# daviddmc/NeSVoR

Measured on AMD Instinct MI355X. Metric: INR train iters/sec (2^20 samples, L=16 hash, 64-wide MLP), higher is better.
Workload: dtype f32 (MLP products evaluated on 2-way fp16 splits of the power-of-two-scaled fp32 operands, fp32 accumulation: error against fp64 at or below the fp32 MFMA chain's; the all-fp32-MFMA rate of the same run is in strict_fp32_mfma)

## Files before the change

include/nesvor_hip.h:

```cpp
#ifndef NESVOR_HIP_H
#define NESVOR_HIP_H

#include <stdint.h>

#ifdef __cplusplus
extern "C" {
#endif

#define NESVOR_MAX_LEVELS 32
#define NESVOR_MAX_MLP_LAYERS 4

int nesvor_hip_abi_version(void);

int nesvor_axisangle2mat_forward(const float* ax, float* mat, int n, void* stream);
int nesvor_axisangle2mat_backward(const float* grad_mat, const float* ax, float* grad_ax, int n, void* stream);
int nesvor_mat2axisangle_forward(const float* mat, float* ax, int n, void* stream);
int nesvor_mat2axisangle_backward(const float* mat, const float* grad_ax, float* grad_mat, int n, void* stream);
int nesvor_axisangle2mat_forward_f64(const double* ax, double* mat, int n, void* stream);
int nesvor_axisangle2mat_backward_f64(const double* grad_mat, const double* ax, double* grad_ax, int n, void* stream);
int nesvor_mat2axisangle_forward_f64(const double* mat, double* ax, int n, void* stream);
int nesvor_mat2axisangle_backward_f64(const double* mat, const double* grad_ax, double* grad_mat, int n, void* stream);

int nesvor_trans_loss(const float* ax, const float* ax_init, float* loss_per_slice, float* grad_ax, int n, void* stream);

// ... 36 lines not shown
                                         const double* psf, const double* grad_slices, const uint8_t* slices_mask,
                                         double* grad_vol, double* grad_transforms, int D, int H, int W, int d_p, int h_p,
                                         int w_p, int n, int h, int w, double res_slice, void* stream);
int nesvor_slice_acq_adjoint_backward_interp_f64(const double* transforms, double* grad_vol, const double* vol_weight,
                                                 const uint8_t* vol_mask, const double* psf, const double* slices,
                                                 const uint8_t* slices_mask, const double* vol, double* grad_slices,
                                                 double* grad_transforms, int D, int H, int W, int d_p, int h_p, int w_p,
                                                 int n, int h, int w, double res_slice, int equalize, void* stream);
int nesvor_slice_acq_forward_f64(const double* transforms, const double* vol, const uint8_t* vol_mask,
                                 const uint8_t* slices_mask, const double* psf, double* slices, double* slices_weight,
                                 int D, int H, int W, int d_p, int h_p, int w_p, int n, int h, int w,
                                 double res_slice, int interp_psf, void* stream);
int nesvor_slice_acq_adjoint_forward_f64(const double* transforms, const double* psf, const double* slices,
                                         const uint8_t* slices_mask, const uint8_t* vol_mask, double* vol, double* vol_weight,
                                         double* scratch, int D, int H, int W, int d_p, int h_p, int w_p, int n, int h, int w,
                                         double res_slice, int equalize, void* stream);
int nesvor_slice_acq_backward_f64(const double* transforms, const double* vol, const uint8_t* vol_mask, const double* psf,
                                  const double* grad_slices, const uint8_t* slices_mask, double* grad_vol,
                                  double* grad_transforms, double* scratch, int D, int H, int W, int d_p, int h_p, int w_p,
                                  int n, int h, int w, double res_slice, void* stream);
int nesvor_slice_acq_adjoint_backward_f64(const double* transforms, double* grad_vol, const double* vol_weight,
                                          const uint8_t* vol_mask, const double* psf, const double* slices,
                                          const uint8_t* slices_mask, const double* vol, double* grad_slices,
                                          double* grad_transforms, int D, int H, int W, int d_p, int h_p, int w_p, int n, int h,
                                          int w, double res_slice, int equalize, void* stream);

typedef struct {
  int32_t n_levels;
  int32_t n_features;
  float scale[NESVOR_MAX_LEVELS];
  uint32_t res[NESVOR_MAX_LEVELS];
  uint32_t size[NESVOR_MAX_LEVELS];
  uint32_t offset[NESVOR_MAX_LEVELS];
  uint32_t hashed[NESVOR_MAX_LEVELS];
} nesvor_grid_t;

#define NESVOR_LAYOUT_ROW_MAJOR 0
#define NESVOR_LAYOUT_FEATURE_MAJOR 1
#define NESVOR_LAYOUT_CLUSTERED 4
#define NESVOR_LAYOUT_UNCLUSTERED 8
#define NESVOR_LAYOUT_DY_SCRATCH 16
#define NESVOR_LAYOUT_MASK 3

int nesvor_hashgrid_forward(const nesvor_grid_t* grid, const float* u, const float* table, float* pe,
                            int64_t N, int layout, void* stream);
int nesvor_hashgrid_forward_bounded(const nesvor_grid_t* grid, const float* u, const float* table, float* pe,
                                    int64_t N, int layout, float* pe_absmax, void* stream);
int64_t nesvor_hashgrid_forward_workspace_bytes(const nesvor_grid_t* grid, int64_t N, int layout);
int nesvor_hashgrid_forward_unclustered(const nesvor_grid_t* grid, const float* u, const float* table, float* pe, int64_t N,
                                        int layout, float* pe_absmax, void* workspace, int64_t workspace_bytes, void* stream);
int64_t nesvor_hashgrid_backward_workspace_bytes(const nesvor_grid_t* grid, int64_t N, const float* queue_scale);
int64_t nesvor_hashgrid_backward_workspace_bytes_ex(const nesvor_grid_t* grid, int64_t N, const float* queue_scale, int layout);
int64_t nesvor_hashgrid_backward_workspace_zero_bytes(void);
int64_t nesvor_hashgrid_backward_overflow_offset(void* workspace);
int nesvor_hashgrid_backward(const nesvor_grid_t* grid, const float* u, const float* table, const float* dpe,
                             float* grad_table, float* grad_u, int64_t N, int layout, void* workspace, int stages,
                             const float* queue_scale, void* stream);

int nesvor_hashgrid_backward_levels(const nesvor_grid_t* grid, const float* u, const float* table, const float* dpe,
                                    float* grad_table, float* grad_u, int64_t N, int layout, void* workspace, int stages,
                                    int level_begin, int level_end, const float* queue_scale, void* stream);
int nesvor_hashgrid_backward_bounded(const nesvor_grid_t* grid, const float* u, const float* table, const float* dpe,
                                     float* grad_table, float* grad_u, int64_t N, int layout, void* workspace, int stages,
                                     int level_begin, int level_end, const float* queue_scale, const float* dy_bound,
                                     void* stream);
int nesvor_hashgrid_backward_atomic(const nesvor_grid_t* grid, const float* u, const float* table, const float* dpe,
                                    float* grad_table, float* grad_u, int64_t N, int layout, void* stream);

int nesvor_psf_transform_forward(const float* mat, const int64_t* slice_idx, const float* xyz, const float* sigma,
                                 const float* noise, const float* bb, float* x, float* u, int B, int S, void* stream);
int nesvor_psf_transform_backward(const float* mat, const int64_t* slice_idx, const float* xyz, const float* sigma,
                                  const float* noise, const float* bb, const float* dx, const float* du, float* dmat,
                                  int B, int S, void* stream);
int nesvor_psf_transform_forward_rng(const float* mat, const int64_t* slice_idx, const float* xyz, const float* sigma,
                                     uint64_t seed, uint64_t offset, const float* bb, float* x, float* u, int B, int S,
                                     void* stream);
int nesvor_psf_transform_forward_rng_gather(const float* mat, const int64_t* slice_idx, const float* xyz, const float* sigma,
                                            uint64_t seed, uint64_t offset, const float* bb, float* x, float* u, int B, int S,
                                            const float* embedding, float* se, int ks, void* stream);
int nesvor_psf_transform_backward_rng(const float* mat, const int64_t* slice_idx, const float* xyz, const float* sigma,
                                      uint64_t seed, uint64_t offset, const float* bb, const float* dx, const float* du,
                                      float* dmat, int B, int S, void* stream);
int nesvor_psf_transform_backward_rng_slices(const float* mat, const int64_t* slice_idx, const float* xyz, const float* sigma,
                                             uint64_t seed, uint64_t offset, const float* bounding_box, const float* dx,
                                             const float* du, float* dpix, float* dmat_slice, int B, int S, void* stream);
int nesvor_psf_noise(uint64_t seed, uint64_t offset, float* out, int64_t n_samples, void* stream);

typedef struct {
  int32_t width;
  int32_t n_hidden;
  int32_t out_dim;
  int32_t k_a, k_b, b_row0;
  int32_t samples_per_pixel;
  int32_t dxa_group_sums;
  int32_t bf16_operands;
  int32_t compact_save;
  const float* weight[NESVOR_MAX_MLP_LAYERS];
  const float* bias[NESVOR_MAX_MLP_LAYERS];
  const float* prep;
  float* y_absmax;
  const void* weight_images;
} nesvor_mlp_t;
#define NESVOR_ABSMAX_SLOTS 16
#define NESVOR_ABSMAX_STRIDE 64
#define NESVOR_ABSMAX_FLOATS (NESVOR_ABSMAX_SLOTS * NESVOR_ABSMAX_STRIDE)
#define NESVOR_MLP_PREP_XA 0
// ... 182 lines not shown
```

nesvor_amd/_lib.py:

```python
import ctypes
import os
from ctypes import POINTER, Structure, c_double, c_float, c_int, c_int32, c_int64, c_uint32, c_uint64, c_void_p

import torch

_HERE = os.path.dirname(os.path.abspath(__file__))
LIB_PATH = os.environ.get("NESVOR_HIP_LIB") or os.path.join(_HERE, "lib", "libnesvor_hip.so")
MAX_LEVELS = 32
ABI_VERSION = 37

LAYOUT_ROW_MAJOR = 0
LAYOUT_FEATURE_MAJOR = 1
STEP_DEFER_JOIN = 8
STEP_BIAS_SUM_STOP = 16
STEP_BIAS_SUM_RESUME = 32
LAYOUT_CLUSTERED = 4
LAYOUT_UNCLUSTERED = 8
LAYOUT_DY_SCRATCH = 16


class GridT(Structure):

    _fields_ = [
        ("n_levels", c_int32),
# ... 105 lines not shown
    "nesvor_hashgrid_forward_workspace_bytes": ([POINTER(GridT), c_int64, c_int], c_int64),
    "nesvor_hashgrid_forward_unclustered": ([POINTER(GridT), _P, _P, _P, c_int64, c_int, _P, _P, c_int64, _P], c_int),
    "nesvor_hashgrid_backward_workspace_bytes": ([POINTER(GridT), c_int64, _P], c_int64),
    "nesvor_hashgrid_backward_workspace_bytes_ex": ([POINTER(GridT), c_int64, _P, c_int], c_int64),
    "nesvor_hashgrid_backward_workspace_zero_bytes": ([], c_int64),
    "nesvor_hashgrid_backward_overflow_offset": ([_P], c_int64),
    "nesvor_hashgrid_backward": ([POINTER(GridT), _P, _P, _P, _P, _P, c_int64, c_int, _P, c_int, _P, _P], c_int),
    "nesvor_hashgrid_backward_levels": ([POINTER(GridT), _P, _P, _P, _P, _P, c_int64, c_int, _P, c_int, c_int, c_int, _P, _P], c_int),
    "nesvor_hashgrid_backward_bounded": ([POINTER(GridT), _P, _P, _P, _P, _P, c_int64, c_int, _P, c_int, c_int, c_int, _P, _P, _P], c_int),
    "nesvor_hashgrid_backward_atomic": ([POINTER(GridT), _P, _P, _P, _P, _P, c_int64, c_int, _P], c_int),
    "nesvor_psf_transform_forward": ([_P] * 8 + [c_int, c_int, _P], c_int),
    "nesvor_psf_transform_backward": ([_P] * 9 + [c_int, c_int, _P], c_int),
    "nesvor_psf_transform_forward_rng_gather": ([_P] * 4 + [c_uint64, c_uint64] + [_P] * 3 + [c_int, c_int, _P, _P, c_int, _P], c_int),
    "nesvor_psf_transform_forward_rng": ([_P] * 4 + [c_uint64, c_uint64] + [_P] * 3 + [c_int, c_int, _P], c_int),
    "nesvor_psf_transform_backward_rng": ([_P] * 4 + [c_uint64, c_uint64] + [_P] * 4 + [c_int, c_int, _P], c_int),
    "nesvor_psf_transform_backward_rng_slices": ([_P] * 4 + [c_uint64, c_uint64] + [_P] * 5 + [c_int, c_int, _P], c_int),
    "nesvor_psf_noise": ([c_uint64, c_uint64, _P, c_int64, _P], c_int),
    "nesvor_mlp_compact_save_ok": ([POINTER(MlpT), c_int64], c_int),
    "nesvor_mlp_bias_free_ok": ([POINTER(MlpT), c_int64], c_int),
    "nesvor_mlp_backward_fused_ok": ([POINTER(MlpT), c_int64], c_int),
    "nesvor_mlp_prepare": ([POINTER(MlpT), _P, _P, _P, c_int64, _P, c_int, _P], c_int),
    "nesvor_mlp_prepare_weights": ([_P, _P, c_int, _P, c_int64, _P, _P], c_int),
    "nesvor_mlp_prepare_weights_images": ([_P, _P, _P, c_int, _P, c_int64, _P, _P], c_int),
    "nesvor_mlp_weight_images_bytes": ([POINTER(MlpT)], c_int64),
    "nesvor_mlp_forward": ([POINTER(MlpT), _P, _P, _P, POINTER(c_void_p), c_int64, _P], c_int),
    "nesvor_mlp_backward": (
        [POINTER(MlpT), _P, _P, _P, POINTER(c_void_p), POINTER(c_void_p), _P, _P, _P, c_int, c_int64, _P],
        c_int,
    ),
    "nesvor_mlp_backward_bounded": (
        [POINTER(MlpT), _P, _P, _P, POINTER(c_void_p), POINTER(c_void_p), _P, _P, _P, c_int, c_int64, _P, _P],
        c_int,
    ),
    "nesvor_mlp_wide_saved_floats": ([POINTER(MlpWideT), c_int64], c_int64),
    "nesvor_mlp_wide_param_count": ([POINTER(MlpWideT)], c_int),
    "nesvor_mlp_wide_forward": ([POINTER(MlpWideT), _P, _P, _P, POINTER(c_void_p), c_int64, _P], c_int),
    "nesvor_mlp_wide_backward": (
        [POINTER(MlpWideT), _P, _P, _P, POINTER(c_void_p), POINTER(c_void_p), _P, _P, _P, c_int, c_int64, _P],
        c_int,
    ),
    "nesvor_mlp_wide_backward_bounded": (
        [POINTER(MlpWideT), _P, _P, _P, POINTER(c_void_p), POINTER(c_void_p), _P, _P, _P, c_int, c_int64, _P, _P],
        c_int,
    ),
    "nesvor_imaging_loss": ([POINTER(LossT), _P], c_int),
    "nesvor_slice_grads_by_slice": ([_P] * 9 + [c_int, c_int, c_int, c_int, _P], c_int),
    "nesvor_slice_grads": ([_P] * 9 + [c_int, c_int, c_int, _P], c_int),
    "nesvor_step_prologue": ([_P] * 5 + [c_int, c_int, _P], c_int),
    "nesvor_step_prologue_pose": ([_P] * 5 + [c_int, c_int, _P, _P, _P, _P], c_int),
    "nesvor_step_epilogue": ([_P] * 6 + [c_float, _P, _P, _P, _P, c_int, c_int, c_float, c_float, _P], c_int),
    "nesvor_step_epilogue_scaled": ([_P] * 6 + [c_float, _P, _P, _P, _P, _P, c_int, c_int, c_float, c_float, _P], c_int),
    "nesvor_hashgrid_backward_adamw": ([POINTER(GridT), _P, _P, _P, _P, _P, c_int64, c_int, _P, c_int, _P, _P, _P, _P, POINTER(AdamwT), _P], c_int),
    "nesvor_hashgrid_backward_adamw_levels": ([POINTER(GridT), _P, _P, _P, _P, _P, c_int64, c_int, _P, c_int, c_int, c_int, _P, _P, _P, _P, POINTER(AdamwT), _P], c_int),
    "nesvor_hashgrid_forward_levels": ([POINTER(GridT), _P, _P, _P, c_int64, c_int, _P, c_int, c_int, _P], c_int),
    "nesvor_adamw_step": (
        [_P, _P, _P, _P, c_int64] + [c_float] * 8 + [c_int, _P],
        c_int,
    ),
    "nesvor_grad_found_inf": ([_P, c_int64, _P, _P], c_int),
    "nesvor_adamw_step_scaled": ([_P, _P, _P, _P, c_int64, c_float, c_double, c_double, c_float, c_float, c_int, c_int, _P, _P], c_int),
    "nesvor_loss_scaler_update": ([_P, _P], c_int),
    "nesvor_loss_scale_weights": ([_P, _P, c_int, _P, _P], c_int),
    "nesvor_sum_rows_multi": ([_P, _P, _P, _P, c_int, c_int, _P], c_int),
    "nesvor_sum_rows": ([_P, _P, c_int, c_int, c_int, _P], c_int),
    "nesvor_step_create": ([POINTER(StepT)], c_void_p),
    "nesvor_step_update": ([_P, POINTER(StepT)], c_int),
    "nesvor_step_destroy": ([_P], None),
    "nesvor_step_join": ([_P, _P], c_int),
    "nesvor_step_set_bias_mean_ranks": ([_P, c_int], c_int),
    "nesvor_step_set_bias_mean_event": ([_P, _P], c_int),
    "nesvor_step_timing": ([_P, c_int], c_int),
    "nesvor_step_timing_read": ([_P, _P], c_int),
    "nesvor_step_run": ([_P, _P, _P, _P, c_uint64, c_uint64, _P, c_int, c_int, POINTER(AdamwT), _P], c_int),
    "nesvor_vvr_similarity": ([_P, c_int, c_int, c_int, _P, _P, _P, _P, c_int64, c_int, _P, _P, _P], c_int),
}


def exported_symbols():
    return list(_SIGNATURES)


def load():
    global _lib
    if _lib is not None:
        return _lib
    if not os.path.exists(LIB_PATH):
        raise RuntimeError(
            f"{LIB_PATH} not found: the HIP backend has not been built. "
            "Run `python -m nesvor_amd.csrc.build` (or __graft_entry__.build()). "
            "There is no CPU fallback for the native ops."
        )
    lib = ctypes.CDLL(LIB_PATH)
    for name, (argtypes, restype) in _SIGNATURES.items():
        fn = getattr(lib, name)
        fn.argtypes = argtypes
        fn.restype = restype
    v = lib.nesvor_hip_abi_version()
    if v != ABI_VERSION:
        raise RuntimeError(f"libnesvor_hip ABI {v} != expected {ABI_VERSION}; rebuild")
    _lib = lib
    return lib


def stream_ptr(device=None):
    return c_void_p(torch.cuda.current_stream(device).cuda_stream)

# ... 60 lines not shown
```

nesvor_amd/csrc/hashgrid.hip:

```cpp
#include <hip/hip_runtime.h>
#include <mutex>
#include <type_traits>
#include <unordered_map>
#include "common.h"
#include "adam.h"
#include "../../include/nesvor_hip.h"

#ifndef NESVOR_ABLATE
#define NESVOR_ABLATE 0
#endif
#define NESVOR_ABL(bit) ((NESVOR_ABLATE & (bit)) != 0)
#ifndef NESVOR_SORT_SPAN
#define NESVOR_SORT_SPAN 256
#endif

namespace {

constexpr uint32_t kPrimeY = 2654435761u;
constexpr uint32_t kPrimeZ = 805459861u;

struct LevelParams {
  float scale;
  uint32_t res, size, offset, hashed;
};

__device__ __forceinline__ LevelParams load_level(const nesvor_grid_t& g, int level) {
  LevelParams p;
  p.scale = g.scale[level];
  p.res = g.res[level];
  p.size = g.size[level];
  p.offset = g.offset[level];
  p.hashed = g.hashed[level];
  return p;
}

__device__ __forceinline__ uint32_t corner_index(const LevelParams& p, uint32_t x, uint32_t y, uint32_t z) {
  if (p.hashed) {
    const uint32_t h = x ^ (y * kPrimeY) ^ (z * kPrimeZ);
    return ((p.size & (p.size - 1)) == 0) ? (h & (p.size - 1)) : (h % p.size);
  }
  uint32_t idx = x + __umul24(y, p.res) + __umul24(z, p.res * p.res);
  if (idx >= p.size) idx %= p.size;
  return idx;
}

__device__ __forceinline__ uint32_t scan32_u32(uint32_t v, int lane) {
#define NESVOR_SCAN_STEP_(SHR)                                                                        \
  v += (uint32_t)__builtin_amdgcn_update_dpp(0, (int)v, 0x110 | (SHR), 0xf, 0xf, true);
  NESVOR_SCAN_STEP_(1) NESVOR_SCAN_STEP_(2) NESVOR_SCAN_STEP_(4) NESVOR_SCAN_STEP_(8)
#undef NESVOR_SCAN_STEP_
  const uint32_t row0 = (uint32_t)__builtin_amdgcn_readlane((int)v, 15);
  return v + ((lane >= 16 && lane < 32) ? row0 : 0u);
}
// ... 535 lines not shown
  x = (x ^ (x << 2)) & 0x09249249u;
  return x;
}

__device__ __forceinline__ unsigned long long to_fixed(float x) {
  const float t = rintf(x * 0x1p-32f);
  const int32_t lo = __float2int_rn(fmaf(-t, 0x1p32f, x));
  return ((unsigned long long)(uint32_t)((int32_t)t + (lo >> 31)) << 32) | (unsigned long long)(uint32_t)lo;
}
#ifndef NESVOR_HG_F64FIX
#define NESVOR_HG_F64FIX 0
#endif
__device__ __forceinline__ unsigned long long to_fixed51(float x, double scale) {
  return (unsigned long long)__double_as_longlong(fma((double)x, scale, 0x1.8p52));
}
__device__ __forceinline__ float from_fixed51(unsigned long long q) {
  const uint32_t lo = (uint32_t)q;
  const int32_t hi = ((int32_t)(uint32_t)(q >> 32) << 13) >> 13;
  return fmaf((float)(hi + (int32_t)(lo >> 31)), 0x1p32f, (float)(int32_t)lo);
}
__device__ __forceinline__ float from_fixed(unsigned long long q) {
  const uint32_t lo = (uint32_t)q;
  return fmaf((float)((int32_t)(q >> 32) + (int32_t)(lo >> 31)), 0x1p32f, (float)(int32_t)lo);
}


#ifndef NESVOR_FIXED32
#define NESVOR_FIXED32 0
#endif

#ifndef NESVOR_HG_SLOTS
#define NESVOR_HG_SLOTS 1024
#endif
#ifndef NESVOR_HG_MINBLOCKS
#define NESVOR_HG_MINBLOCKS 4
#endif
#ifndef NESVOR_HG_SPATIAL
#define NESVOR_HG_SPATIAL 1
#endif
#ifndef NESVOR_HG_TIMELINE
#define NESVOR_HG_TIMELINE 0
#endif
#if NESVOR_HG_TIMELINE
constexpr int kTlWgs = 64, kTlMarks = 96;
__device__ unsigned long long g_hg_timeline[kTlWgs][kTlMarks];
#define HG_TICK(site)                                                                                              \
  do {                                                                                                             \
    if (blockIdx.x < (unsigned)kTlWgs && threadIdx.x == 0 && tl_n < kTlMarks)                                      \
      g_hg_timeline[blockIdx.x][tl_n++] = ((unsigned long long)(site) << 56) | (__builtin_amdgcn_s_memtime() & 0x00FFFFFFFFFFFFFFull); \
  } while (0)
#else
#define HG_TICK(site) do { } while (0)
#endif
template <int F, int LAYOUT, bool INPUT_GRAD, bool MERGE, bool BOUND = false>
__global__ __launch_bounds__(256, F <= 2 ? NESVOR_HG_MINBLOCKS : (F == 4 ? 3 : 2)) void hashgrid_bwd_aggregate(const nesvor_grid_t g, const BwdPlan plan,
                                                              const float* __restrict__ u,
                                                              const float* __restrict__ table,
                                                              const float* __restrict__ dpe,
                                                              float* __restrict__ grad_table,
                                                              float* __restrict__ grad_u, uint32_t* __restrict__ tails,
                                                              uint32_t* __restrict__ tails_next,
                                                              uint32_t* __restrict__ records, int64_t N,
                                                              const float* __restrict__ dy_bound,
                                                              uint8_t* __restrict__ order,
                                                              int order_mode,
                                                              const uint32_t* __restrict__ perm,
                                                              int dy_by_slot) {
  for (uint32_t t = blockIdx.x * 256u + threadIdx.x; t < (uint32_t)kSubQueues * kTailStride; t += gridDim.x * 256u) tails_next[t] = 0u;
  constexpr bool kPack = (F == 2) && (NESVOR_FIXED32 != 0);
  constexpr bool kPerLevel = kPack && (NESVOR_FIXED32 >= 2);
  constexpr int kWords = kPack ? 1 : F;
  __shared__ uint32_t bcount[kMaxChunks];
  __shared__ __attribute__((aligned(16))) uint32_t bb_raw[4 * kMaxChunks];
  uint4* const bbase4 = reinterpret_cast<uint4*>(bb_raw);
  uint2(*const bbase)[kMaxChunks] = reinterpret_cast<uint2(*)[kMaxChunks]>(bb_raw);
  __shared__ uint32_t sortbuf[256];
  constexpr int kSlots = F <= 2 ? NESVOR_HG_SLOTS : (F == 4 ? 512 : 256);
  constexpr uint32_t kEmpty = 0xFFFFFFFFu;
  constexpr uint32_t kKeyMask = (1u << 27) - 1u;
  constexpr int kMaxGroup = 8;
  __shared__ __attribute__((aligned(16))) uint32_t tkeys[kSlots];
  __shared__ __attribute__((aligned(16))) unsigned long long tvals[kSlots * kWords];
  __shared__ __attribute__((aligned(16))) float tcache[INPUT_GRAD && MERGE ? kSlots * F : 1];
  __shared__ float gmax[4];
  __shared__ uint32_t lmax_bits[NESVOR_MAX_LEVELS + 1];
  __shared__ float lscale[NESVOR_MAX_LEVELS + 1][2];
  __shared__ uint32_t merge_stat[2];
  __shared__ uint32_t slots_log2;
  __shared__ uint32_t merge_off;
  __shared__ uint32_t prev_cnt;
  __shared__ float ubox[4][6];
  __shared__ uint32_t lbox[NESVOR_MAX_LEVELS + 1][8];
  __shared__ uint32_t lwin[NESVOR_MAX_LEVELS + 1];
  __shared__ uint32_t slot_off[NESVOR_MAX_LEVELS + 1], bkt_off[NESVOR_MAX_LEVELS + 1], grp_end[NESVOR_MAX_LEVELS + 1];
  __shared__ uint32_t rnd_slots[NESVOR_MAX_LEVELS + 1], rnd_bkts[NESVOR_MAX_LEVELS + 1];
  __shared__ uint32_t lpar[NESVOR_MAX_LEVELS + 1][8];
  __shared__ int32_t box_end_s;
  const int tid = threadIdx.x, lane = tid & 63;
  const int64_t base = (int64_t)blockIdx.x * 256;
  const int E = g.n_levels * F;
#if NESVOR_HG_TIMELINE
  int tl_n = 0;
  if (blockIdx.x < (unsigned)kTlWgs && tid == 0) for (int k = 0; k < kTlMarks; ++k) g_hg_timeline[blockIdx.x][k] = 0ull;
#endif
  HG_TICK(0);
  const int level_end = plan.level_end;
  const uint32_t sub = (uint32_t)__builtin_amdgcn_s_getreg((3 << 11) | (0 << 6) | 20) & (plan.n_sub - 1u);
  if (tid < kMaxChunks) bcount[tid] = 0;
  for (int t = tid; t < kSlots; t += 256) tkeys[t] = kEmpty;
  for (int t = tid; t < kSlots * kWords; t += 256) tvals[t] = 0ull;
  if (tid < 2) merge_stat[tid] = 0;
  if (tid == 0) { merge_off = MERGE ? 0u : 1u; slots_log2 = __builtin_ctz(kSlots); prev_cnt = 0u; }
  if constexpr (kPerLevel) {
    if (tid <= NESVOR_MAX_LEVELS) lmax_bits[tid] = 0u;
  }

  uint32_t sv;
  {
    const int64_t s0_ = base + tid;
    uint32_t code = 0x00ffffffu;
    if (s0_ < N) {
      const int64_t i0 = perm != nullptr ? (int64_t)perm[s0_] : s0_;
      const LevelParams pf = load_level(g, g.n_levels - 1);
      const CellPos c = locate(pf, u[3 * i0], u[3 * i0 + 1], u[3 * i0 + 2]);
      code = spread3(c.gx) | (spread3(c.gy) << 1) | (spread3(c.gz) << 2);
    }
    sv = (code << 8) | (uint32_t)tid;
    if (order_mode == 2) sv = (uint32_t)order[base + tid];
    else
// ... 272 lines not shown
#pragma unroll
        for (int f = 0; f < F; ++f) {
          v[f] = (NESVOR_HG_F64FIX != 0 ? from_fixed51(w[f]) : from_fixed(w[f])) * finv;
          tvals[f * kSlots + slot] = 0ull;
        }
      }
    }
    return any;
  };

  float dy_a[F], dy_b[F];
  int level = plan.level_begin;
  load_dy(level, dy_a);
  if (level + 1 < level_end) load_dy(level + 1, dy_b);

  constexpr int NRB = kSlots / 256;
  if constexpr (MERGE) {
    auto fill_keys = [&](int ra, int rb, float (&feat)[NRB][F]) __attribute__((always_inline)) {
      const uint32_t total = sgpr(rnd_slots[ra]);
#pragma unroll
      for (int j = 0; j < NRB; ++j) {
        const uint32_t slot = (uint32_t)j * 256u + (uint32_t)tid;
#pragma unroll
        for (int f = 0; f < F; ++f) feat[j][f] = 0.f;
        if (slot < total) {
          int lv = ra;
          for (int l = ra + 1; l < rb; ++l) lv = slot >= slot_off[l] ? l : lv;
          const uint32_t local = slot - slot_off[lv];
          const uint32_t nx = lbox[lv][3] + 2u, nxy = nx * (lbox[lv][4] + 2u);
          const uint32_t z = (uint32_t)(((float)local + 0.5f) * (1.f / (float)nxy));
          const uint32_t r = local - __umul24(z, nxy);
          const uint32_t y = (uint32_t)(((float)r + 0.5f) * (1.f / (float)nx));
          LevelParams pl;
          pl.scale = 0.f; pl.res = lpar[lv][0]; pl.size = lpar[lv][1]; pl.offset = lpar[lv][2]; pl.hashed = lpar[lv][3];
          const uint32_t key = corner_index(pl, lbox[lv][0] + (r - __umul24(y, nx)), lbox[lv][1] + y, lbox[lv][2] + z);
          tkeys[slot] = ((uint32_t)lv << 27) | key;
          if constexpr (INPUT_GRAD) load_feat<F>(table + ((size_t)pl.offset + key) * F, feat[j]);
        }
      }
    };
    auto store_feat = [&](int ra, const float (&feat)[NRB][F]) __attribute__((always_inline)) {
      if constexpr (INPUT_GRAD) {
        const uint32_t total = sgpr(rnd_slots[ra]);
#pragma unroll
        for (int j = 0; j < NRB; ++j) {
          const uint32_t slot = (uint32_t)j * 256u + (uint32_t)tid;
          if (slot < total) {
#pragma unroll
            for (int f = 0; f < F; ++f) tcache[slot * F + f] = feat[j][f];
          }
        }
      }
    };
    auto insert_round = [&](int ra, int rb) __attribute__((always_inline)) {
#pragma unroll 1
      for (int lv = ra; lv < rb; ++lv) {
        uint32_t idx_unused[8], s0, nx, nxy;
        float val[8][F];
        bool tail;
        prepare(std::true_type{}, lv, dy_a, idx_unused, s0, nx, nxy, val, tail);
#pragma unroll
        for (int f = 0; f < F; ++f) dy_a[f] = dy_b[f];
        if (lv + 2 < level_end) load_dy(lv + 2, dy_b);
        const float fs_lv = scale_of((uint32_t)lv);
        if (!NESVOR_ABL(4) && tail) {
#pragma unroll
          for (int k = 0; k < 8; ++k) slot_add(s0 + (k & 1) + ((k >> 1) & 1) * nx + (k >> 2) * nxy, val[k], fs_lv);
        }
      }
    };

    if (level < box_end) {
      int ra = level, rb = (int)sgpr(grp_end[level]);
      {
        float feat[NRB][F];
        fill_keys(ra, rb, feat);
        store_feat(ra, feat);
      }
      if constexpr (INPUT_GRAD) __syncthreads();
      HG_TICK(4);
      insert_round(ra, rb);
      HG_TICK(5);
      uint32_t rkey[NRB], rmeta[NRB], rank[NRB], rmask = 0;
      float rval[NRB][F];
      bool have_prev = false;
      for (;;) {
        __syncthreads();
        HG_TICK(0x20 | ra);
        if (have_prev && !NESVOR_ABL(8)) {
#pragma unroll
          for (int j = 0; j < NRB; ++j) {
            if (!(rmask & (1u << j))) continue;
            const uint4 bb = bbase4[rmeta[j] & 0xFFu];
            const uint32_t pos = bb.x + rank[j];
            if (pos < bb.z) {
              uint32_t* r = records + ((size_t)bb.y + pos) * (1 + F);
              r[0] = rkey[j];
#pragma unroll
              for (int f = 0; f < F; ++f) r[1 + f] = __float_as_uint(rval[j][f]);
            } else {
              atomicAdd(&tails[kOverflowBase + (rmeta[j] >> 8)], 1u);
#pragma unroll
              for (int f = 0; f < F; ++f) atomicAdd(grad_table + ((size_t)lpar[rmeta[j] >> 8][2] + rkey[j]) * F + f, rval[j][f]);
            }
          }
        }
        const int na = rb, nb_ = na < box_end ? (int)sgpr(grp_end[na]) : na;
        const bool next_box = na < box_end;
        const uint32_t n_slots = sgpr(rnd_slots[ra]);
        uint32_t lk[NRB];
#pragma unroll
        for (int j = 0; j < NRB; ++j) lk[j] = tkeys[j * 256 + tid];
        float nfeat[NRB][F];
        if (next_box) {
          fill_keys(na, nb_, nfeat);
        } else {
#pragma unroll
          for (int j = 0; j < NRB; ++j) tkeys[j * 256 + tid] = kEmpty;
        }
        rmask = 0;
        uint32_t n_last = 0;
// ... 738 lines not shown
    for (int idx = tid; idx < kGatherPts * E; idx += 256) {
      const int q = idx / E, e = idx - q * E;
      if (i0 + q < N) rows[(size_t)rank[q] * E + e] = tile[q * (E + 1) + e];
    }
  }
}
__global__ __launch_bounds__(256) void scatter_pe_rows_kernel(const float* __restrict__ rows, SortBufs s, float* __restrict__ pe, int64_t N, int E) {
  extern __shared__ float tile[];
  __shared__ uint32_t rank[kGatherPts];
  const int tid = threadIdx.x;
  const int64_t i0 = (int64_t)blockIdx.x * kGatherPts;
  const bool ok = i0 + tid < N;
  if (ok) {
    const unsigned long long w = s.where[i0 + tid];
    rank[tid] = s.first[(uint32_t)(w >> 32)] + (uint32_t)w;
  }
  __syncthreads();
  if ((E & 3) == 0) {
    const int E4 = E >> 2;
    for (int idx = tid; idx < kGatherPts * E4; idx += 256) {
      const int q = idx / E4, e = (idx - q * E4) * 4;
      if (i0 + q < N) {
        const float4 v = *reinterpret_cast<const float4*>(rows + (size_t)rank[q] * E + e);
        float* t = tile + q * (E + 1) + e;
        t[0] = v.x; t[1] = v.y; t[2] = v.z; t[3] = v.w;
      }
    }
  } else {
    for (int idx = tid; idx < kGatherPts * E; idx += 256) {
      const int q = idx / E, e = idx - q * E;
      if (i0 + q < N) tile[q * (E + 1) + e] = rows[(size_t)rank[q] * E + e];
    }
  }
  __syncthreads();
  if (ok) {
    for (int e = 0; e < E; ++e) pe[(size_t)e * N + i0 + tid] = tile[tid * (E + 1) + e];
  }
}
inline int sort_points(const float* u, int64_t N, uint32_t* base, hipStream_t st) {
  const SortPlan p = sort_plan(N);
  const SortBufs s = sort_bufs(base, N, p);
  hipError_t e = hipMemsetAsync(s.count, 0, sizeof(uint32_t) * (p.n_cells + 1), st);
  if (e != hipSuccess) return (int)e;
  hipLaunchKernelGGL(sort_place_kernel, dim3((unsigned)((N + 255) / 256)), dim3(256), 0, st, u, N, p, s);
  static std::once_flag raised;
  constexpr size_t kScanLds = sizeof(uint32_t) * (32768 + 32768 / 32);
  std::call_once(raised, []() { (void)hipFuncSetAttribute(reinterpret_cast<const void*>(sort_scan_kernel), hipFuncAttributeMaxDynamicSharedMemorySize, (int)kScanLds); });
  hipLaunchKernelGGL(sort_scan_kernel, dim3(1), dim3(1024), kScanLds, st, p, s);
  const uint64_t n_threads = (uint64_t)p.n_cells * p.cap + (uint64_t)((N + 255) / 256) * 256;
  hipLaunchKernelGGL(sort_compact_kernel, dim3((unsigned)((n_threads + 255) / 256)), dim3(256), 0, st, p, s);
  return (int)hipGetLastError();
}

template <int F, int LAYOUT>
int launch_bwd_owner(const nesvor_grid_t* g, const float* u, const float* table, const float* dpe, float* gt,
                     float* gu, int64_t N, void* workspace, int stages, int level_begin, int level_end, const float* queue_scale,
                     const float* dy_bound, const OwnerAdam* adam, hipStream_t st, int hints = 0) {
  const bool unclustered = (hints & NESVOR_LAYOUT_UNCLUSTERED) != 0;
  if constexpr (LAYOUT == NESVOR_LAYOUT_FEATURE_MAJOR) {
    if (unclustered && (hints & NESVOR_LAYOUT_DY_SCRATCH) && (stages & 1))
      return launch_bwd_owner<F, NESVOR_LAYOUT_ROW_MAJOR>(g, u, table, dpe, gt, gu, N, workspace, stages, level_begin, level_end, queue_scale,
                                                          dy_bound, adam, st, hints | 0x10000);
  }
  BwdPlan plan;
  uint64_t n_rec;
  if (!make_plan(g, N, &plan, &n_rec, queue_scale)) return (int)hipErrorInvalidValue;
  plan.level_begin = level_begin; plan.level_end = level_end;
  plan.accumulate_u = (stages & 8) ? 1 : 0;
  const int par = tails_parity(workspace, (stages & 1) && !(stages & 4));
  uint32_t* tails = reinterpret_cast<uint32_t*>(reinterpret_cast<char*>(workspace) + (par ? kTailBytes : 0));
  uint32_t* tails_next = reinterpret_cast<uint32_t*>(reinterpret_cast<char*>(workspace) + (par ? 0 : kTailBytes));
  uint32_t* records = reinterpret_cast<uint32_t*>(reinterpret_cast<char*>(workspace) + kHeadBytes);
  uint8_t* order = reinterpret_cast<uint8_t*>(records) + n_rec * (1 + F) * sizeof(uint32_t);
  const int order_mode = (stages & 4) ? 2 : 1;
  uint32_t* const perm_buf = reinterpret_cast<uint32_t*>((reinterpret_cast<uintptr_t>(order) + (uintptr_t)((N + 255) / 256) * 256 + 255) & ~(uintptr_t)255);
  const uint32_t* const perm = unclustered ? perm_buf : nullptr;
  dim3 grid((unsigned)((N + 255) / 256)), block(256);
  hipError_t e;
  int dy_by_slot = 0;
  if (!(stages & 1)) goto owner_stage;
  if (unclustered && order_mode == 1) {
    const int se = sort_points(u, N, perm_buf, st);
    if (se) return se;
  }
  if (hints & 0x10000) {
    const int E = g->n_levels * F;
    float* rows = reinterpret_cast<float*>(reinterpret_cast<char*>(perm_buf) + ((sort_bytes(N) + 255) & ~(uint64_t)255));
    if (order_mode == 1) {
      const size_t lds = sizeof(float) * kGatherPts * (E + 1);
      if (lds > 48 * 1024) {
        static std::mutex mu;
        static size_t raised = 0;
        std::lock_guard<std::mutex> lock(mu);
        if (lds > raised) {
          e = hipFuncSetAttribute(reinterpret_cast<const void*>(gather_dy_rows_kernel), hipFuncAttributeMaxDynamicSharedMemorySize, (int)lds);
          if (e != hipSuccess) return (int)e;
          raised = lds;
        }
      }
      hipLaunchKernelGGL(gather_dy_rows_kernel, dim3((unsigned)((N + kGatherPts - 1) / kGatherPts)), dim3(256), lds, st, dpe,
                         sort_bufs(perm_buf, N, sort_plan(N)), rows, N, E);
    }
    dpe = rows;
    dy_by_slot = 1;
  }
  {
    static const bool merge = []() { const char* e = getenv("NESVOR_HASHGRID_MERGE"); return e == nullptr || atoi(e) != 0; }();
#define NESVOR_LAUNCH_AGG(IG, MG, BD)                                                                                     \
    hipLaunchKernelGGL((hashgrid_bwd_aggregate<F, LAYOUT, IG, MG, BD>), grid, block, 0, st, *g, plan, u, table, dpe, gt, gu, \
                       tails, tails_next, records, N, dy_bound, order, order_mode, perm, dy_by_slot)
    const bool bounded = dy_bound != nullptr && merge;
    if (gu != nullptr) { if (bounded) NESVOR_LAUNCH_AGG(true, true, true); else if (merge) NESVOR_LAUNCH_AGG(true, true, false); else NESVOR_LAUNCH_AGG(true, false, false); }
    else { if (bounded) NESVOR_LAUNCH_AGG(false, true, true); else if (merge) NESVOR_LAUNCH_AGG(false, true, false); else NESVOR_LAUNCH_AGG(false, false, false); }
#undef NESVOR_LAUNCH_AGG
  }
  e = hipGetLastError();
  if (e != hipSuccess) return (int)e;
owner_stage:
  if (stages & 2) {
    static const int coalesced = []() { const char* e = getenv("NESVOR_OWNER_COALESCED"); return e == nullptr ? 1 : atoi(e); }();
    OwnerAdam oa{};
    static const uint32_t want = []() { const char* e = getenv("NESVOR_OWNER_STRIDE"); return e ? (uint32_t)atoi(e) : 1u; }();
    const uint32_t wg_base = NESVOR_OWNER_FINE_FIRST ? 0u : owner_grid(g, plan, 0, plan.level_begin);
    const uint32_t og = NESVOR_OWNER_FINE_FIRST ? owner_grid(g, plan) : owner_grid(g, plan, plan.level_begin, plan.level_end);
    if (og == 0u) return (int)hipGetLastError();
    uint32_t id_stride = want < 1u ? 1u : want;
    auto gcd = [](uint32_t a, uint32_t b) { while (b) { const uint32_t t = a % b; a = b; b = t; } return a; };
    while (id_stride > 1u && gcd(id_stride, og) != 1u) ++id_stride;
    if (adam != nullptr) {
      oa = *adam;
      oa.done = reinterpret_cast<uint32_t*>(reinterpret_cast<char*>(workspace) + 2 * kTailBytes);
      hipLaunchKernelGGL((hashgrid_bwd_owner<F, true, true>), dim3(og), dim3(kOwnerThreads), 0, st, *g, plan, tails, records, gt, oa, id_stride, wg_base);
    } else if (coalesced)
      hipLaunchKernelGGL((hashgrid_bwd_owner<F, true>), dim3(og), dim3(kOwnerThreads), 0, st, *g, plan, tails, records, gt, oa, id_stride, wg_base);
    else
      hipLaunchKernelGGL((hashgrid_bwd_owner<F, false>), dim3(og), dim3(kOwnerThreads), 0, st, *g, plan, tails, records, gt, oa, id_stride, wg_base);
  }
  return (int)hipGetLastError();
}

inline uint64_t fwd_ws_bytes(const nesvor_grid_t* g, int64_t N, int layout) {
  const uint64_t n_pad = (uint64_t)((N + 255) / 256) * 256;
  uint64_t b = 256 + ((sort_bytes(N) + 255) & ~(uint64_t)255);
  if ((layout & NESVOR_LAYOUT_MASK) == NESVOR_LAYOUT_FEATURE_MAJOR) b += n_pad * (uint64_t)(g->n_levels * g->n_features) * sizeof(float);
  return b;
}
template <int F, int LAYOUT>
int launch_fwd_unclustered(const nesvor_grid_t* g, const float* u, const float* table, float* pe, int64_t N, float* pe_absmax,
                           void* workspace, hipStream_t st) {
  uint32_t* const perm_buf = reinterpret_cast<uint32_t*>((reinterpret_cast<uintptr_t>(workspace) + 255) & ~(uintptr_t)255);
  const int se = sort_points(u, N, perm_buf, st);
  if (se) return se;
  float* rows = nullptr;
  const int E = g->n_levels * F;
  if constexpr (LAYOUT == NESVOR_LAYOUT_FEATURE_MAJOR)
    rows = reinterpret_cast<float*>(reinterpret_cast<char*>(perm_buf) + ((sort_bytes(N) + 255) & ~(uint64_t)255));
  hipLaunchKernelGGL((hashgrid_fwd_cloud<F, LAYOUT>), dim3((unsigned)((N + 255) / 256)), dim3(256), 0, st, *g, u, table, pe, N, pe_absmax,
                     (const uint32_t*)perm_buf, rows);
  if constexpr (LAYOUT == NESVOR_LAYOUT_FEATURE_MAJOR) {
    const size_t lds = sizeof(float) * kGatherPts * (E + 1);
    if (lds > 48 * 1024) {
      static std::mutex mu;
      static size_t raised = 0;
      std::lock_guard<std::mutex> lock(mu);
      if (lds > raised) {
        const hipError_t e = hipFuncSetAttribute(reinterpret_cast<const void*>(scatter_pe_rows_kernel), hipFuncAttributeMaxDynamicSharedMemorySize, (int)lds);
        if (e != hipSuccess) return (int)e;
// ... 86 lines not shown
  if (grid->n_levels <= 0 || grid->n_levels > NESVOR_MAX_LEVELS) return (int)hipErrorInvalidValue;
  if (level_begin < 0 || level_end > grid->n_levels || level_begin >= level_end) return (int)hipErrorInvalidValue;
  layout &= NESVOR_LAYOUT_MASK;
  DISPATCH_F_LAYOUT(launch_fwd_levels, grid, u, table, pe, N, pe_absmax, level_begin, level_end, (hipStream_t)stream);
}

extern "C" int64_t nesvor_hashgrid_forward_workspace_bytes(const nesvor_grid_t* grid, int64_t N, int layout) {
  if (grid == nullptr || N <= 0) return 0;
  if (!(layout & NESVOR_LAYOUT_UNCLUSTERED)) return 0;
  return (int64_t)fwd_ws_bytes(grid, N, layout);
}

extern "C" int nesvor_hashgrid_forward_unclustered(const nesvor_grid_t* grid, const float* u, const float* table, float* pe,
                                                   int64_t N, int layout, float* pe_absmax, void* workspace, int64_t workspace_bytes,
                                                   void* stream) {
  if (N <= 0) return 0;
  if (grid->n_levels <= 0 || grid->n_levels > NESVOR_MAX_LEVELS) return (int)hipErrorInvalidValue;
  if (N >= ((int64_t)1 << 32)) return (int)hipErrorInvalidValue;
  if (workspace == nullptr || workspace_bytes < (int64_t)fwd_ws_bytes(grid, N, layout)) return (int)hipErrorInvalidValue;
  layout &= NESVOR_LAYOUT_MASK;
  DISPATCH_F_LAYOUT(launch_fwd_unclustered, grid, u, table, pe, N, pe_absmax, workspace, (hipStream_t)stream);
}

extern "C" int nesvor_hashgrid_backward_atomic(const nesvor_grid_t* grid, const float* u, const float* table,
                                               const float* dpe, float* grad_table, float* grad_u, int64_t N,
                                               int layout, void* stream) {
  if (N <= 0) return 0;
  if (grid->n_levels <= 0 || grid->n_levels > NESVOR_MAX_LEVELS) return (int)hipErrorInvalidValue;
  layout &= NESVOR_LAYOUT_MASK;
  DISPATCH_F_LAYOUT(launch_bwd, grid, u, table, dpe, grad_table, grad_u, N, (hipStream_t)stream);
}

extern "C" int64_t nesvor_hashgrid_backward_workspace_bytes_ex(const nesvor_grid_t* grid, int64_t N, const float* queue_scale, int layout) {
  int64_t base = nesvor_hashgrid_backward_workspace_bytes(grid, N, queue_scale);
  if (base <= 0) return base;
  if (!(layout & NESVOR_LAYOUT_UNCLUSTERED)) base -= (int64_t)((sort_bytes(N) + 255) & ~(uint64_t)255);
  if ((layout & NESVOR_LAYOUT_MASK) == NESVOR_LAYOUT_FEATURE_MAJOR && (layout & NESVOR_LAYOUT_UNCLUSTERED) && (layout & NESVOR_LAYOUT_DY_SCRATCH))
    return base + 256 + (int64_t)((N + 255) / 256) * 256 * grid->n_levels * grid->n_features * (int64_t)sizeof(float);
  return base;
}

extern "C" int64_t nesvor_hashgrid_backward_workspace_bytes(const nesvor_grid_t* grid, int64_t N, const float* queue_scale) {
  if (N <= 0) return 0;
  BwdPlan plan;
  uint64_t n_rec;
  if (grid->n_levels <= 0 || grid->n_levels > NESVOR_MAX_LEVELS) return -1;
  if (!make_plan(grid, N, &plan, &n_rec, queue_scale)) return -1;
  if (plan.n_buckets > kOverflowBase) return -1;
  return (int64_t)(kHeadBytes + n_rec * (1 + grid->n_features) * sizeof(uint32_t) + (uint64_t)((N + 255) / 256) * 256 + 256 + ((sort_bytes(N) + 255) & ~(uint64_t)255));
}

extern "C" int64_t nesvor_hashgrid_backward_workspace_zero_bytes(void) { return (int64_t)kHeadBytes; }

#if NESVOR_HG_TIMELINE
extern "C" int nesvor_debug_hg_timeline(unsigned long long* dst_host) {
  return (int)hipMemcpyFromSymbol(dst_host, HIP_SYMBOL(g_hg_timeline), sizeof(unsigned long long) * kTlWgs * kTlMarks);
}
#endif

extern "C" int64_t nesvor_hashgrid_backward_overflow_offset(void* workspace) {
  return (int64_t)(tails_parity(workspace, false) ? kTailBytes : 0) + (int64_t)kOverflowBase * (int64_t)sizeof(uint32_t);
}

extern "C" int nesvor_hashgrid_backward(const nesvor_grid_t* grid, const float* u, const float* table,
                                        const float* dpe, float* grad_table, float* grad_u, int64_t N, int layout,
                                        void* workspace, int stages, const float* queue_scale, void* stream) {
  if (N <= 0) return 0;
  if (grid->n_levels <= 0 || grid->n_levels > NESVOR_MAX_LEVELS) return (int)hipErrorInvalidValue;
  if (workspace == nullptr || (stages & 3) == 0) return (int)hipErrorInvalidValue;
  const int hints = layout & (NESVOR_LAYOUT_UNCLUSTERED | NESVOR_LAYOUT_DY_SCRATCH);
  layout &= NESVOR_LAYOUT_MASK;
  DISPATCH_F_LAYOUT(launch_bwd_owner, grid, u, table, dpe, grad_table, grad_u, N, workspace, stages & 3, 0, grid->n_levels,
                    queue_scale, nullptr, nullptr, (hipStream_t)stream, hints);
}

extern "C" int nesvor_hashgrid_backward_levels(const nesvor_grid_t* grid, const float* u, const float* table,
                                               const float* dpe, float* grad_table, float* grad_u, int64_t N, int layout,
                                               void* workspace, int stages, int level_begin, int level_end,
                                               const float* queue_scale, void* stream) {
  if (N <= 0) return 0;
  if (grid->n_levels <= 0 || grid->n_levels > NESVOR_MAX_LEVELS) return (int)hipErrorInvalidValue;
  if (workspace == nullptr || (stages & 3) == 0) return (int)hipErrorInvalidValue;
  if (level_begin < 0 || level_end > grid->n_levels || level_begin >= level_end) return (int)hipErrorInvalidValue;
  const int hints = layout & (NESVOR_LAYOUT_UNCLUSTERED | NESVOR_LAYOUT_DY_SCRATCH);
  layout &= NESVOR_LAYOUT_MASK;
  DISPATCH_F_LAYOUT(launch_bwd_owner, grid, u, table, dpe, grad_table, grad_u, N, workspace, stages, level_begin, level_end,
                    queue_scale, nullptr, nullptr, (hipStream_t)stream, hints);
}

extern "C" int nesvor_hashgrid_backward_bounded(const nesvor_grid_t* grid, const float* u, const float* table,
                                                const float* dpe, float* grad_table, float* grad_u, int64_t N, int layout,
                                                void* workspace, int stages, int level_begin, int level_end,
                                                const float* queue_scale, const float* dy_bound, void* stream) {
  if (N <= 0) return 0;
  if (grid->n_levels <= 0 || grid->n_levels > NESVOR_MAX_LEVELS) return (int)hipErrorInvalidValue;
  if (workspace == nullptr || (stages & 3) == 0) return (int)hipErrorInvalidValue;
  if (level_begin < 0 || level_end > grid->n_levels || level_begin >= level_end) return (int)hipErrorInvalidValue;
  const int hints = layout & (NESVOR_LAYOUT_UNCLUSTERED | NESVOR_LAYOUT_DY_SCRATCH);
  layout &= NESVOR_LAYOUT_MASK;
  DISPATCH_F_LAYOUT(launch_bwd_owner, grid, u, table, dpe, grad_table, grad_u, N, workspace, stages, level_begin, level_end,
                    queue_scale, dy_bound, nullptr, (hipStream_t)stream, hints);
}

extern "C" int nesvor_hashgrid_backward_adamw(const nesvor_grid_t* grid, const float* u, float* table, const float* dpe,
                                              float* grad_table, float* grad_u, int64_t N, int layout, void* workspace,
                                              int stages, const float* queue_scale, const float* dy_bound, float* exp_avg,
// ... 25 lines not shown
```

Baseline: 1058.

## Compact sparse tail inserts into per-wave LDS strips before slot atomics

In the merge aggregation kernel of the hashgrid backward, levels where only a few lanes of a wave hold a tail entry no longer issue eight scattered slot atomics from those lanes. The lanes write their corner values and packed slot offsets into a per-wave shared-memory strip, and the whole wave then flushes the strip with all 64 lanes doing the atomics. The goal is to avoid idle lanes during the sparse insert phase. In exchange the sort buffer grows into larger strips, which raises LDS use and may lower occupancy, and wave-level fences are added. The new path is on by default and can be switched off at runtime.

```diff
diff --git a/include/nesvor_hip.h b/include/nesvor_hip.h
--- a/include/nesvor_hip.h
+++ b/include/nesvor_hip.h
@@ -112,6 +112,7 @@
 int64_t nesvor_hashgrid_backward_workspace_bytes(const nesvor_grid_t* grid, int64_t N, const float* queue_scale);
 int64_t nesvor_hashgrid_backward_workspace_bytes_ex(const nesvor_grid_t* grid, int64_t N, const float* queue_scale, int layout);
 int64_t nesvor_hashgrid_backward_workspace_zero_bytes(void);
+int nesvor_hashgrid_dense_inserts(int on);
 int64_t nesvor_hashgrid_backward_overflow_offset(void* workspace);
 int nesvor_hashgrid_backward(const nesvor_grid_t* grid, const float* u, const float* table, const float* dpe,
                              float* grad_table, float* grad_u, int64_t N, int layout, void* workspace, int stages,
diff --git a/nesvor_amd/_lib.py b/nesvor_amd/_lib.py
--- a/nesvor_amd/_lib.py
+++ b/nesvor_amd/_lib.py
@@ -181,6 +181,7 @@
     "nesvor_step_epilogue_scaled": ([_P] * 6 + [c_float, _P, _P, _P, _P, _P, c_int, c_int, c_float, c_float, _P], c_int),
     "nesvor_hashgrid_backward_adamw": ([POINTER(GridT), _P, _P, _P, _P, _P, c_int64, c_int, _P, c_int, _P, _P, _P, _P, POINTER(AdamwT), _P], c_int),
     "nesvor_hashgrid_backward_adamw_levels": ([POINTER(GridT), _P, _P, _P, _P, _P, c_int64, c_int, _P, c_int, c_int, c_int, _P, _P, _P, _P, POINTER(AdamwT), _P], c_int),
+    "nesvor_hashgrid_dense_inserts": ([c_int], c_int),
     "nesvor_hashgrid_forward_levels": ([POINTER(GridT), _P, _P, _P, c_int64, c_int, _P, c_int, c_int, _P], c_int),
     "nesvor_adamw_step": (
         [_P, _P, _P, _P, c_int64] + [c_float] * 8 + [c_int, _P],
diff --git a/nesvor_amd/csrc/hashgrid.hip b/nesvor_amd/csrc/hashgrid.hip
--- a/nesvor_amd/csrc/hashgrid.hip
+++ b/nesvor_amd/csrc/hashgrid.hip
@@ -1,4 +1,5 @@
 #include <hip/hip_runtime.h>
+#include <atomic>
 #include <mutex>
 #include <type_traits>
 #include <unordered_map>
@@ -640,7 +641,10 @@
 #else
 #define HG_TICK(site) do { } while (0)
 #endif
-template <int F, int LAYOUT, bool INPUT_GRAD, bool MERGE, bool BOUND = false>
+#ifndef NESVOR_HG_DENSE_INSERT
+#define NESVOR_HG_DENSE_INSERT 1
+#endif
+template <int F, int LAYOUT, bool INPUT_GRAD, bool MERGE, bool BOUND = false, bool DENSE = false>
 __global__ __launch_bounds__(256, F <= 2 ? NESVOR_HG_MINBLOCKS : (F == 4 ? 3 : 2)) void hashgrid_bwd_aggregate(const nesvor_grid_t g, const BwdPlan plan,
                                                               const float* __restrict__ u,
                                                               const float* __restrict__ table,
@@ -662,7 +666,13 @@
   __shared__ __attribute__((aligned(16))) uint32_t bb_raw[4 * kMaxChunks];
   uint4* const bbase4 = reinterpret_cast<uint4*>(bb_raw);
   uint2(*const bbase)[kMaxChunks] = reinterpret_cast<uint2(*)[kMaxChunks]>(bb_raw);
-  __shared__ uint32_t sortbuf[256];
+  constexpr bool kDense = DENSE && MERGE && !kPack && F <= 2;
+  constexpr int kItemVals = 8 * F;
+  constexpr int kStripItems = 240 / kItemVals;
+  constexpr int kStripWords = kDense ? 4 * kStripItems * (kItemVals + 1) : 256;
+  static_assert(kStripWords >= 256 && 64 % kItemVals == 0, "the strips hold the sort buffer; a pass of 64 lanes takes whole items");
+  __shared__ __attribute__((aligned(16))) uint32_t strip_raw[kStripWords];
+  uint32_t* const sortbuf = strip_raw;
   constexpr int kSlots = F <= 2 ? NESVOR_HG_SLOTS : (F == 4 ? 512 : 256);
   constexpr uint32_t kEmpty = 0xFFFFFFFFu;
   constexpr uint32_t kKeyMask = (1u << 27) - 1u;
@@ -1041,7 +1051,29 @@
         }
       }
     };
+    float* const strip_val = reinterpret_cast<float*>(strip_raw) + (tid >> 6) * (kStripItems * kItemVals);
+    uint32_t* const strip_hdr = strip_raw + 4 * kStripItems * kItemVals + (tid >> 6) * kStripItems;
+    static_assert(!kDense || kSlots <= 2048, "a strip header packs slot | nx << 11 | nxy << 21");
+    auto strip_flush = [&](uint32_t n) __attribute__((always_inline)) {
+      __builtin_amdgcn_fence(__ATOMIC_RELEASE, "wavefront");
+      __builtin_amdgcn_wave_barrier();
+      const uint32_t k = ((uint32_t)lane / (uint32_t)F) & 7u, f = (uint32_t)lane % (uint32_t)F;
+      const uint32_t mx = k & 1u, my = (k & 2u) ? 1023u : 0u, mz = (k & 4u) ? 2047u : 0u;
+      unsigned long long* const tv = tvals + f * kSlots;
+      const uint32_t total = n * (uint32_t)kItemVals;
+#pragma unroll 1
+      for (uint32_t e = (uint32_t)lane; e < total; e += 64u) {
+        const uint32_t h = strip_hdr[e / (uint32_t)kItemVals];
+        const float v = strip_val[e];
+        const uint32_t slot = (h & 2047u) + mx + ((h >> 11) & my) + ((h >> 21) & mz);
+        if constexpr (NESVOR_HG_F64FIX != 0) atomicAdd(&tv[slot], to_fixed51(v, (double)fscale));
+        else atomicAdd(&tv[slot], to_fixed(v * fscale));
+      }
+      __builtin_amdgcn_fence(__ATOMIC_ACQ_REL, "wavefront");
+      __builtin_amdgcn_wave_barrier();
+    };
     auto insert_round = [&](int ra, int rb) __attribute__((always_inline)) {
+      uint32_t n_items = 0;
 #pragma unroll 1
       for (int lv = ra; lv < rb; ++lv) {
         uint32_t idx_unused[8], s0, nx, nxy;
@@ -1052,10 +1084,35 @@
         for (int f = 0; f < F; ++f) dy_a[f] = dy_b[f];
         if (lv + 2 < level_end) load_dy(lv + 2, dy_b);
         const float fs_lv = scale_of((uint32_t)lv);
-        if (!NESVOR_ABL(4) && tail) {
+        bool direct = true;
+        if constexpr (kDense) {
+          const unsigned long long tmask = __ballot(tail);
+          const uint32_t nt = (uint32_t)__popcll(tmask);
+          direct = nt > (uint32_t)kStripItems;
+          if (!direct && !NESVOR_ABL(4)) {
+            if (n_items + nt > (uint32_t)kStripItems) { strip_flush(n_items); n_items = 0; }
+            if (tail) {
+              const uint32_t pos = n_items + __builtin_amdgcn_mbcnt_hi((uint32_t)(tmask >> 32), __builtin_amdgcn_mbcnt_lo((uint32_t)tmask, 0u));
+              strip_hdr[pos] = s0 | (nx << 11) | (nxy << 21);
+              float4* const row = reinterpret_cast<float4*>(strip_val + pos * (uint32_t)kItemVals);
+              if constexpr (F == 1) {
+                row[0] = make_float4(val[0][0], val[1][0], val[2][0], val[3][0]);
+                row[1] = make_float4(val[4][0], val[5][0], val[6][0], val[7][0]);
+              } else {
+#pragma unroll
+                for (int q = 0; q < 4; ++q) row[q] = make_float4(val[2 * q][0], val[2 * q][1], val[2 * q + 1][0], val[2 * q + 1][1]);
+              }
+            }
+            n_items += nt;
+          }
+        }
+        if (direct && !NESVOR_ABL(4) && tail) {
 #pragma unroll
           for (int k = 0; k < 8; ++k) slot_add(s0 + (k & 1) + ((k >> 1) & 1) * nx + (k >> 2) * nxy, val[k], fs_lv);
         }
+      }
+      if constexpr (kDense) {
+        if (n_items) strip_flush(n_items);
       }
     };
 
@@ -1900,6 +1957,8 @@
   return (int)hipGetLastError();
 }
 
+std::atomic<int> g_dense_inserts{NESVOR_HG_DENSE_INSERT != 0 ? 1 : 0};
+
 template <int F, int LAYOUT>
 int launch_bwd_owner(const nesvor_grid_t* g, const float* u, const float* table, const float* dpe, float* gt,
                      float* gu, int64_t N, void* workspace, int stages, int level_begin, int level_end, const float* queue_scale,
@@ -1954,13 +2013,21 @@
   }
   {
     static const bool merge = []() { const char* e = getenv("NESVOR_HASHGRID_MERGE"); return e == nullptr || atoi(e) != 0; }();
+#define NESVOR_LAUNCH_AGG_(IG, MG, BD, DN)                                                                                \
+    hipLaunchKernelGGL((hashgrid_bwd_aggregate<F, LAYOUT, IG, MG, BD, DN>), grid, block, 0, st, *g, plan, u, table, dpe, gt, gu, \
+                       tails, tails_next, records, N, dy_bound, order, order_mode, perm, dy_by_slot)
 #define NESVOR_LAUNCH_AGG(IG, MG, BD)                                                                                     \
-    hipLaunchKernelGGL((hashgrid_bwd_aggregate<F, LAYOUT, IG, MG, BD>), grid, block, 0, st, *g, plan, u, table, dpe, gt, gu, \
-                       tails, tails_next, records, N, dy_bound, order, order_mode, perm, dy_by_slot)
+    do {                                                                                                                  \
+      if constexpr (MG && F <= 2 && NESVOR_FIXED32 == 0) {                                                                \
+        if (g_dense_inserts.load(std::memory_order_relaxed)) NESVOR_LAUNCH_AGG_(IG, MG, BD, true);                        \
+        else NESVOR_LAUNCH_AGG_(IG, MG, BD, false);                                                                       \
+      } else NESVOR_LAUNCH_AGG_(IG, MG, BD, false);                                                                       \
+    } while (0)
     const bool bounded = dy_bound != nullptr && merge;
     if (gu != nullptr) { if (bounded) NESVOR_LAUNCH_AGG(true, true, true); else if (merge) NESVOR_LAUNCH_AGG(true, true, false); else NESVOR_LAUNCH_AGG(true, false, false); }
     else { if (bounded) NESVOR_LAUNCH_AGG(false, true, true); else if (merge) NESVOR_LAUNCH_AGG(false, true, false); else NESVOR_LAUNCH_AGG(false, false, false); }
 #undef NESVOR_LAUNCH_AGG
+#undef NESVOR_LAUNCH_AGG_
   }
   e = hipGetLastError();
   if (e != hipSuccess) return (int)e;
@@ -2153,6 +2220,10 @@
 
 extern "C" int64_t nesvor_hashgrid_backward_workspace_zero_bytes(void) { return (int64_t)kHeadBytes; }
 
+extern "C" int nesvor_hashgrid_dense_inserts(int on) {
+  return on < 0 ? g_dense_inserts.load(std::memory_order_relaxed) : g_dense_inserts.exchange(on != 0 ? 1 : 0, std::memory_order_relaxed);
+}
+
 #if NESVOR_HG_TIMELINE
 extern "C" int nesvor_debug_hg_timeline(unsigned long long* dst_host) {
   return (int)hipMemcpyFromSymbol(dst_host, HIP_SYMBOL(g_hg_timeline), sizeof(unsigned long long) * kTlWgs * kTlMarks);
```

After: 1062 (median of 6 runs). Within noise of the previous version (+0.4%).
